# Deci-AI/super-gradients

Measured on NVIDIA H100. Metric: images/sec YOLO-NAS-S 640 bf16 train, higher is better.
Workload: dtype bf16

## Files before the change

include/sgb200.h:

```cpp
#ifndef SGB200_H_
#define SGB200_H_

#include <stdint.h>

#ifdef __cplusplus
extern "C" {
#endif

#define SGB_OK 0
#define SGB_E_INVALID (-1)
#define SGB_E_UNSUPPORTED (-2)
#define SGB_E_CUDA (-3)
#define SGB_E_ARCH (-4)

#define SGB_ACT_NONE 0
#define SGB_ACT_RELU 1
#define SGB_ACT_SILU 2

typedef uint16_t sgb_bf16;

typedef struct SgbConvDesc {
  int32_t N, H, W, C;
  int32_t K, R, S;
  int32_t P, Q;
  int32_t stride, pad;
  int32_t x_pitch, x_off;
  int32_t y_pitch, y_off;
  int32_t up2;
  int32_t centre_from;
} SgbConvDesc;

typedef struct SgbEpilogue {
  const float* scale;
  const float* shift;
  const sgb_bf16* residual;
  double* stats;
  int32_t stats_repl;
  int32_t act;
  int32_t out_f32;
} SgbEpilogue;

const char* sgb_last_error(void);
int sgb_version(void);
int sgb_check_device(void);
int64_t sgb_sm100_launches(void);
int64_t sgb_conv_halo_launches(void);
void sgb_conv_force_im2col(int on);
int64_t sgb_conv_wgrad_halo_launches(void);
void sgb_conv_wgrad_force_im2col(int on);

int sgb_conv_fprop(const SgbConvDesc* d, const sgb_bf16* x, const sgb_bf16* w_krsc, void* y, const SgbEpilogue* ep,
                   void* stream);
int sgb_conv_dgrad(const SgbConvDesc* d, const sgb_bf16* dy, const sgb_bf16* w_crsk, sgb_bf16* dx, int accumulate,
                   void* stream);
int sgb_conv_wgrad(const SgbConvDesc* d, const sgb_bf16* x, const sgb_bf16* dy, float* dw_krsc, void* stream);
int sgb_weight_prepare(const float* w_oihw, int K, int C, int R, int S, int c_pad, sgb_bf16* w_krsc, sgb_bf16* w_crsk,
                       const float* scale, int add_identity, void* stream);
int sgb_wgrad_to_oihw(const float* dw_krsc, int K, int C, int R, int S, int c_pad, float* g_oihw, int accumulate,
                      void* stream);
typedef struct SgbWeightItem {
  const float* w;
  const float* scale;
  sgb_bf16* krsc;
  sgb_bf16* crsk;
  int32_t K, C, R, S, c_pad, add_identity;
  int32_t kp, koff, etaps, etap;
  int64_t start;
} SgbWeightItem;
typedef struct SgbWgradItem {
  const float* dw;
  float* g;
  int32_t K, C, R, S, c_pad, accumulate;
  int64_t start;
} SgbWgradItem;
int sgb_weight_prepare_batch(const SgbWeightItem* items_dev, int n_items, int64_t total, void* stream);
typedef struct SgbAlphaItem {
  const float* dw1;
  const float* w1;
  const float* alpha;
  const float* dab;
  const float* bias1;
  float* g_w1;
  float* g_bias;
  float* g_alpha;
  int32_t K, C, c_pad, pad_;
} SgbAlphaItem;
int sgb_qarep_alpha_finish_batch(const SgbAlphaItem* items_dev, int n_items, void* stream);
int sgb_wgrad_to_oihw_batch(const SgbWgradItem* items_dev, int n_items, int64_t total, void* stream);
int sgb_convt2x2_fprop(const SgbConvDesc* d, const sgb_bf16* x_small, const sgb_bf16* w_up, const float* bias,
                       sgb_bf16* y_up, void* stream);

int sgb_nchw_f32_to_nhwc_bf16(const float* x, int N, int C, int H, int W, sgb_bf16* y, int y_pitch, int y_off, int c_out,
                              void* stream);
int sgb_stem_patches_f32(const float* x, int N, int C, int H, int W, int R, int stride, int pad, sgb_bf16* y, int P, int Q, int c_out,
                         void* stream);
int sgb_nhwc_bf16_to_nchw_f32(const sgb_bf16* x, int N, int C, int H, int W, int x_pitch, int x_off, float* y,
                              void* stream);

typedef struct SgbBnDesc {
  int64_t M;
  int32_t C;
  int32_t x_pitch, x_off;
  int32_t y_pitch, y_off;
  int32_t r_pitch, r_off;
  float eps, momentum;
  int32_t act;
  int32_t stats_repl;
  int32_t dy_pitch, dy_off;
  int64_t hw;
  const float* sample_scale;
  int32_t dy2_split, dy2_pitch, dy2_off, dy2_reserved;
  const void* dy2;
  const double* count;
  float param_scale;
  int32_t count_reserved;
} SgbBnDesc;
int sgb_bn_act_fwd(const SgbBnDesc* d, const sgb_bf16* x, const double* stats, const float* gamma, const float* beta,
                   float* running_mean, float* running_var, const sgb_bf16* residual, sgb_bf16* y, float* save_mean,
                   float* save_rstd, void* stream);
int sgb_bn_act_infer(const SgbBnDesc* d, const sgb_bf16* x, const float* gamma, const float* beta,
                     const float* running_mean, const float* running_var, const sgb_bf16* residual, sgb_bf16* y,
                     void* stream);
int sgb_bn_act_bwd_reduce(const SgbBnDesc* d, const sgb_bf16* dy, const sgb_bf16* x, const sgb_bf16* y, const float* gamma,
                          const float* beta, const float* save_mean, const float* save_rstd, double* sums, void* stream);
int sgb_bn_act_bwd_apply(const SgbBnDesc* d, const sgb_bf16* dy, const sgb_bf16* x, const sgb_bf16* y,
                         const float* gamma, const float* beta, const float* save_mean, const float* save_rstd,
                         const double* sums, sgb_bf16* dx, sgb_bf16* dresidual, float* dgamma, float* dbeta, void* stream);
int sgb_channel_stats(const sgb_bf16* x, int64_t M, int C, int pitch, int off, double* stats, void* stream);

typedef struct SgbQarepDesc {
  int64_t M;
  int32_t C;
// ... 295 lines not shown
```

super_gradients_b200/csrc/capi.cu:

```cuda
#include <cstdarg>
#include <cstdio>

#include "common.cuh"
#include "conv_sm100.h"
#include "sm100_host.h"

static thread_local char g_err[512] = "";

void sgb_set_error(const char* fmt, ...) {
  va_list ap;
  va_start(ap, fmt);
  vsnprintf(g_err, sizeof(g_err), fmt, ap);
  va_end(ap);
}

int sgb_cuda_check(cudaError_t e, const char* what) {
  if (e == cudaSuccess) return SGB_OK;
  sgb_set_error("%s: %s", what, cudaGetErrorString(e));
  return SGB_E_CUDA;
}

extern "C" const char* sgb_last_error(void) { return g_err; }
extern "C" int sgb_version(void) { return 100; }
extern "C" int sgb_check_device(void) {
  int dev = 0;
  if (int rc = sgb_cuda_check(cudaGetDevice(&dev), "cudaGetDevice")) return rc;
  cudaDeviceProp prop;
  if (int rc = sgb_cuda_check(cudaGetDeviceProperties(&prop, dev), "cudaGetDeviceProperties")) return rc;
  if (prop.major != 9) {
    sgb_set_error("libsgb200 is built for sm_90a only; device is sm_%d%d", prop.major, prop.minor);
    return SGB_E_ARCH;
  }
  return SGB_OK;
}

extern "C" int64_t sgb_sm100_launches(void) { return (int64_t)sm100::launch_count(); }
extern "C" int64_t sgb_conv_halo_launches(void) { return (int64_t)sm100::halo_launch_count(); }
extern "C" void sgb_conv_force_im2col(int on) { sm100::force_im2col(on != 0); }
extern "C" int64_t sgb_conv_wgrad_halo_launches(void) { return (int64_t)sm100::wgrad_halo_launch_count(); }
extern "C" void sgb_conv_wgrad_force_im2col(int on) { sm100::wgrad_force_im2col(on != 0); }
```

super_gradients_b200/csrc/conv_sm100.cu:

```cuda
#include <cuda.h>

#include <cstdlib>
#include <cstring>

#include "common.cuh"
#include "conv_sm100.h"
#include "sm100_host.h"
#include "sm100_ptx.cuh"

namespace sm100 {

constexpr int BLOCK_M = 128;
constexpr int NUM_THREADS = 384;
constexpr int CONSUMER_THREADS = 256;
constexpr int MAX_STAGES = 8;

struct Params {
  int M;
  int N;
  int C;
  int KC;
  int n_tiles;
  int stages;
  int P, Q;
// ... 289 lines not shown
    asm volatile("fence.mbarrier_init.release.cluster;" ::: "memory");
    asm volatile("fence.proxy.async.shared::cta;" ::: "memory");
  }
  if (p.stats)
    for (int i = threadIdx.x; i < 4 * p.N; i += NUM_THREADS) s_stats[i] = 0.f;
  __syncthreads();

  if (warp == 0) {
    if (elect_one()) {
      mbar_expect_tx(b_bar, (uint32_t)(8 * off + ksteps) * b_box);
      for (int bt = 0; bt < 9; ++bt)
        for (int ks = 0; ks < (bt == CENTRE_TAP ? ksteps : off); ++ks)
          tma_load_2d(sb + (uint32_t)(bt * ksteps + ks) * b_box, &map_b, b_bar, bt * p.b_cols_per_tap + 16 * ks, nt * BN);
      const uint32_t a_tx = (uint32_t)(p.C / 8) * (HALO_H * HALO_W * 16);
      int stg = 0;
      uint32_t par = 1;
      for (int mt = mt0; mt < m_tiles; mt += mt_step) {
        const int n_img = mt / p.halo_thw;
        const int rem = mt - n_img * p.halo_thw;
        const int th = rem / p.halo_tw, tw = rem - th * p.halo_tw;
        mbar_wait(empty_bar(stg), par);
        const uint32_t sa = sa0 + stg * a_stage;
        mbar_expect_tx(full_bar(stg), a_tx);
        for (int cg = 0; cg < p.C / 8; ++cg)
          tma_load_tiled_4d(sa + (uint32_t)cg * HALO_CG_BYTES, &map_a, full_bar(stg), 8 * cg, tw * HALO_TILE - 1, th * HALO_TILE - 1,
                            n_img);
        if (++stg == p.stages) {
          stg = 0;
          par ^= 1;
        }
      }
    }
  } else if (warp >= 4) {
    const int wg = (warp >> 2) - 1;
    const int wq = warp & 3;
    float acc[BN / 2];
    mbar_wait(b_bar, 0);
    for (int j = wg, mt = mt0 + wg * mt_step; mt < m_tiles; j += 2, mt += 2 * mt_step) {
      const int stg = j % p.stages;
      mbar_wait(full_bar(stg), (uint32_t)(j / p.stages) & 1u);
      const uint32_t sa = sa0 + stg * a_stage;
      wgmma_fence();
      int t = off > 0 ? 0 : CENTRE_TAP;
      uint32_t sa_t = sa + (uint32_t)((t / 3) * HALO_W + t % 3) * 16u, sb_t = sb + (uint32_t)(p.tap_b[t] * ksteps) * b_box;
      for (int k = 0, ks = 0, nk = 8 * off + ksteps; k < nk; ++k) {
        const uint64_t da = smem_desc_noswizzle(sa_t + (uint32_t)(2 * ks) * HALO_CG_BYTES, HALO_CG_BYTES, HALO_W * 16);
        const uint64_t db = smem_desc(sb_t + (uint32_t)ks * b_box, 32, 16u, 256u);
        mma_kk<BN>(acc, da, db, k != 0);
        if (++ks == (t == CENTRE_TAP ? ksteps : off) && ++t < 9) {
          ks = 0;
          sa_t = sa + (uint32_t)((t / 3) * HALO_W + t % 3) * 16u;
          sb_t = sb + (uint32_t)(p.tap_b[t] * ksteps) * b_box;
        }
      }
      wgmma_commit();
      wgmma_wait<0>();
      fence_regs(acc);
      __syncwarp();
      if (lane == 0) mbar_arrive(empty_bar(stg));

      const int n_img = mt / p.halo_thw;
      const int rem = mt - n_img * p.halo_thw;
      const int th = rem / p.halo_tw, tw = rem - th * p.halo_tw;
      const int ow = tw * HALO_TILE + (lane >> 2);
      long long orow[2];
      bool row_ok[2];
#pragma unroll
      for (int h = 0; h < 2; ++h) {
        const int oh = th * HALO_TILE + 2 * wq + h;
        row_ok[h] = oh < p.P && ow < p.Q;
        orow[h] = row_ok[h] ? ((long long)n_img * p.P + oh) * p.Q + ow : 0;
      }
      tile_epilogue<BN, 4>(p, acc, orow, row_ok, nt, wg, wq, lane, s_part + wg * 4 * 2 * BN, s_stats + wg * 2 * p.N);
    }
  }
  __syncthreads();
  if (p.stats) {
    for (int i = threadIdx.x; i < 2 * p.N; i += NUM_THREADS) s_stats[i] += s_stats[2 * p.N + i];
    __syncthreads();
  }
  flush_stats(p, s_stats);
}

struct WParams {
  int K, C;
  int R, S, stride, pad, P, Q;
  int npix;
  int CB;
  int n_ctiles;
  int rb_all, rb_off;
  int items;
  int pix_per_cta;
  int stages;
  int cpad;
  float* dw;
  int halo_tw, halo_thw, tiles, tiles_per_cta;
};
constexpr int WPIX = 64;

__host__ __device__ __forceinline__ int wgrad_row_blocks(const WParams& p, int tap) {
  return p.R * p.S == 9 && tap != CENTRE_TAP ? p.rb_off : p.rb_all;
}

template <int NB>
__global__ void __launch_bounds__(NUM_THREADS, 1)
wgrad_wgmma_kernel(const __grid_constant__ CUtensorMap map_dy, const __grid_constant__ CUtensorMap map_x, const WParams p) {
  extern __shared__ __align__(1024) unsigned char smem_raw[];
  const uint32_t smem_base = (smem_u32(smem_raw) + 1023u) & ~1023u;
  const uint32_t a_bytes = 2 * WPIX * 128;
  const uint32_t b_box = WPIX * p.CB * 2;
  const int boxes = NB / p.CB;
  const uint32_t stage_bytes = a_bytes + (uint32_t)boxes * b_box;
  const uint32_t ctrl = smem_base + p.stages * stage_bytes;
  auto full_bar = [&](int s) { return ctrl + 8u * s; };
  auto empty_bar = [&](int s) { return ctrl + 8u * (MAX_STAGES + s); };

  const int warp = threadIdx.x >> 5, lane = threadIdx.x & 31;
  int w = blockIdx.x;
  const int split = w / (p.items * p.n_ctiles);
  w -= split * p.items * p.n_ctiles;
  int tap = 0, tap_items = (wgrad_row_blocks(p, 0) + 1) / 2;
  while (w >= tap_items * p.n_ctiles) {
    w -= tap_items * p.n_ctiles;
    tap_items = (wgrad_row_blocks(p, ++tap) + 1) / 2;
  }
  const int ctile = w / tap_items, item = w - ctile * tap_items;
  const bool shared_rows = 2 * item + 1 == wgrad_row_blocks(p, tap);
  const int row0 = 128 * item;
  const int pix0 = split * p.pix_per_cta;
  const int pix1 = min(pix0 + p.pix_per_cta, p.npix);
  const int n_iters = (pix1 - pix0 + WPIX - 1) / WPIX;

  if (threadIdx.x == 0) {
    for (int s = 0; s < p.stages; ++s) {
      mbar_init(full_bar(s), 1);
      mbar_init(empty_bar(s), shared_rows ? 4 : 8);
    }
    asm volatile("fence.mbarrier_init.release.cluster;" ::: "memory");
    asm volatile("fence.proxy.async.shared::cta;" ::: "memory");
  }
  __syncthreads();

  if (n_iters > 0) {
    if (warp == 0) {
      if (elect_one()) {
        const int pq = p.P * p.Q;
        const int r = tap / p.S, s = tap - r * p.S;
        int stg = 0;
        uint32_t par = 1;
        for (int it = 0; it < n_iters; ++it) {
          mbar_wait(empty_bar(stg), par);
          const uint32_t sa = smem_base + stg * stage_bytes, sb = sa + a_bytes;
          mbar_expect_tx(full_bar(stg), (shared_rows ? a_bytes / 2 : a_bytes) + (uint32_t)boxes * b_box);
          const int pix = pix0 + it * WPIX;
          tma_load_2d(sa, &map_dy, full_bar(stg), row0, pix);
          if (!shared_rows) tma_load_2d(sa + WPIX * 128, &map_dy, full_bar(stg), row0 + 64, pix);
          const int n_img = pix / pq;
          const int rem = pix - n_img * pq;
          const int p0 = rem / p.Q, q0 = rem - p0 * p.Q;
          const int w0 = q0 * p.stride - p.pad, h0 = p0 * p.stride - p.pad;
          for (int bx = 0; bx < boxes; ++bx)
            tma_load_im2col_4d(sb + (uint32_t)bx * b_box, &map_x, full_bar(stg), ctile * NB + bx * p.CB, w0, h0, n_img, (uint16_t)s,
                               (uint16_t)r);
          if (++stg == p.stages) {
            stg = 0;
            par ^= 1;
// ... 107 lines not shown
      if (ko < p.K) {
        float* drow = p.dw + (long long)ko * row_len + tap0 * p.cpad + ctile * NB + 2 * (lane & 3);
#pragma unroll
        for (int t = 0; t < NT; ++t)
#pragma unroll
          for (int j = 0; j < NB / 8; ++j)
            asm volatile("red.global.add.v2.f32 [%0], {%1, %2};" ::"l"(drow + t * p.cpad + 8 * j), "f"(acc[t][4 * j + 2 * h]),
                         "f"(acc[t][4 * j + 2 * h + 1])
                         : "memory");
      }
    }
  }
}

template <int NB>
__global__ void __launch_bounds__(NUM_THREADS, 1)
wgrad3x3_halo_kernel(const __grid_constant__ CUtensorMap map_dy, const __grid_constant__ CUtensorMap map_x, const WParams p) {
  extern __shared__ __align__(1024) unsigned char smem_raw[];
  const uint32_t smem_base = (smem_u32(smem_raw) + 1023u) & ~1023u;
  constexpr uint32_t a_bytes = WH_A_BYTES, stage_bytes = wgrad_halo_stage_bytes(NB);
  const uint32_t ctrl = smem_base + p.stages * stage_bytes;
  auto full_bar = [&](int s) { return ctrl + 8u * s; };
  auto empty_bar = [&](int s) { return ctrl + 8u * (MAX_STAGES + s); };

  const int warp = threadIdx.x >> 5;
  const int items = p.rb_all * p.n_ctiles;
  const int split = blockIdx.x / items, item = blockIdx.x - split * items;
  const int ctile = item / p.rb_all, rb = item - ctile * p.rb_all;
  const bool all_taps = rb < p.rb_off;
  const int t0 = split * p.tiles_per_cta, t1 = min(t0 + p.tiles_per_cta, p.tiles);

  if (threadIdx.x == 0) {
    for (int s = 0; s < p.stages; ++s) {
      mbar_init(full_bar(s), 1);
      mbar_init(empty_bar(s), 8);
    }
    asm volatile("fence.mbarrier_init.release.cluster;" ::: "memory");
    asm volatile("fence.proxy.async.shared::cta;" ::: "memory");
  }
  __syncthreads();

  if (warp == 0) {
    if (elect_one()) {
      const uint32_t tx = a_bytes + (NB / 8) * (HALO_H * HALO_W * 16);
      int stg = 0;
      uint32_t par = 1;
      for (int mt = t0; mt < t1; ++mt) {
        const int n_img = mt / p.halo_thw;
        const int rem = mt - n_img * p.halo_thw;
        const int th = rem / p.halo_tw, tw = rem - th * p.halo_tw;
        mbar_wait(empty_bar(stg), par);
        const uint32_t sa = smem_base + stg * stage_bytes;
        mbar_expect_tx(full_bar(stg), tx);
        tma_load_tiled_4d(sa, &map_dy, full_bar(stg), 64 * rb, tw * HALO_TILE, th * HALO_TILE, n_img);
        for (int cg = 0; cg < NB / 8; ++cg)
          tma_load_tiled_4d(sa + a_bytes + (uint32_t)cg * HALO_CG_BYTES, &map_x, full_bar(stg), ctile * NB + 8 * cg,
                            tw * HALO_TILE - 1, th * HALO_TILE - 1, n_img);
        if (++stg == p.stages) {
          stg = 0;
          par ^= 1;
        }
      }
    }
  } else if (warp >= 4) {
    const int wg = (warp >> 2) - 1;
    const uint32_t ring = smem_base, bars = ctrl;
    if (!all_taps && wg == 0)
      wgrad_halo_consume<NB, 1>(p, ring, bars, t0, t1, CENTRE_TAP, rb, ctile);
    else if (!all_taps)
      wgrad_halo_consume<NB, 0>(p, ring, bars, t0, t1, 0, rb, ctile);
    else if (wg == 0)
      wgrad_halo_consume<NB, 5>(p, ring, bars, t0, t1, 0, rb, ctile);
    else
      wgrad_halo_consume<NB, 4>(p, ring, bars, t0, t1, 5, rb, ctile);
  }
}

EncodeTiledFn g_tiled = nullptr;
EncodeIm2colFn g_im2col = nullptr;
int g_num_sms = 0;
long long g_launches = 0;
long long g_halo_launches = 0;
long long g_wgrad_halo_launches = 0;
bool g_force_im2col = false;
bool g_wgrad_force_im2col = false;
long long launch_count() { return g_launches; }
long long halo_launch_count() { return g_halo_launches; }
long long wgrad_halo_launch_count() { return g_wgrad_halo_launches; }
void force_im2col(bool on) { g_force_im2col = on; }
void wgrad_force_im2col(bool on) { g_wgrad_force_im2col = on; }

int init_driver() {
  if (g_tiled && g_im2col) return SGB_OK;
  cudaDriverEntryPointQueryResult qres;
  void* fn = nullptr;
  if (cudaGetDriverEntryPoint("cuTensorMapEncodeTiled", &fn, cudaEnableDefault, &qres) != cudaSuccess || !fn) {
    sgb_set_error("cuTensorMapEncodeTiled entry point not found");
    return SGB_E_CUDA;
  }
  g_tiled = (EncodeTiledFn)fn;
  fn = nullptr;
  if (cudaGetDriverEntryPoint("cuTensorMapEncodeIm2col", &fn, cudaEnableDefault, &qres) != cudaSuccess || !fn) {
    sgb_set_error("cuTensorMapEncodeIm2col entry point not found");
    return SGB_E_CUDA;
  }
  g_im2col = (EncodeIm2colFn)fn;
  int dev = 0;
  cudaGetDevice(&dev);
  cudaDeviceGetAttribute(&g_num_sms, cudaDevAttrMultiProcessorCount, dev);
  return SGB_OK;
}

CUtensorMapSwizzle swizzle_for(int kc) {
  return kc == 64 ? CU_TENSOR_MAP_SWIZZLE_128B : (kc == 32 ? CU_TENSOR_MAP_SWIZZLE_64B : CU_TENSOR_MAP_SWIZZLE_32B);
}

bool supported(const Problem& q) {
  if (q.C % 16 != 0 || q.b_rows % 8 != 0) return false;
  if (!((q.R == 1 && q.S == 1) || (q.R == 3 && q.S == 3))) return false;
  if (q.stride != 1 && q.stride != 2) return false;
  if (q.a_pitch % 8 != 0 || q.y_pitch % 8 != 0 || q.y_off % 8 != 0) return false;
  if (((uintptr_t)q.a & 15) || ((uintptr_t)q.b & 15) || ((uintptr_t)q.y & 15)) return false;
  if ((long long)q.N * q.P * q.Q >= (1ll << 31)) return false;
  if (q.b_rows > 4096) return false;
  return true;
}

namespace {

template <class Fn>
struct Variant {
  int bn;
  Fn fn;
  int regs;
  bool ready;
};
typedef void (*ConvFn)(const CUtensorMap, const CUtensorMap, const Params);
typedef void (*WgradFn)(const CUtensorMap, const CUtensorMap, const WParams);
Variant<ConvFn> g_conv[] = {{16, conv_wgmma_kernel<16, false>, 0, false},   {32, conv_wgmma_kernel<32, false>, 0, false},
                            {48, conv_wgmma_kernel<48, false>, 0, false},   {64, conv_wgmma_kernel<64, false>, 0, false},
                            {96, conv_wgmma_kernel<96, false>, 0, false},   {128, conv_wgmma_kernel<128, false>, 0, false}};
Variant<ConvFn> g_conv_skip[] = {{16, conv_wgmma_kernel<16, true>, 0, false},   {32, conv_wgmma_kernel<32, true>, 0, false},
                                 {48, conv_wgmma_kernel<48, true>, 0, false},   {64, conv_wgmma_kernel<64, true>, 0, false},
                                 {96, conv_wgmma_kernel<96, true>, 0, false},   {128, conv_wgmma_kernel<128, true>, 0, false}};
Variant<ConvFn> g_halo[] = {{16, conv3x3_halo_kernel<16, false>, 0, false},   {32, conv3x3_halo_kernel<32, false>, 0, false},
                            {48, conv3x3_halo_kernel<48, false>, 0, false},   {64, conv3x3_halo_kernel<64, false>, 0, false},
                            {96, conv3x3_halo_kernel<96, false>, 0, false},   {128, conv3x3_halo_kernel<128, false>, 0, false}};
Variant<ConvFn> g_halo_skip[] = {{16, conv3x3_halo_kernel<16, true>, 0, false},   {32, conv3x3_halo_kernel<32, true>, 0, false},
                                 {48, conv3x3_halo_kernel<48, true>, 0, false},   {64, conv3x3_halo_kernel<64, true>, 0, false},
                                 {96, conv3x3_halo_kernel<96, true>, 0, false},   {128, conv3x3_halo_kernel<128, true>, 0, false}};
Variant<WgradFn> g_wgrad[] = {{16, wgrad_wgmma_kernel<16>, 0, false}, {32, wgrad_wgmma_kernel<32>, 0, false},
                              {48, wgrad_wgmma_kernel<48>, 0, false}, {64, wgrad_wgmma_kernel<64>, 0, false},
                              {96, wgrad_wgmma_kernel<96>, 0, false}, {128, wgrad_wgmma_kernel<128>, 0, false}};
Variant<WgradFn> g_wgrad_halo[] = {{16, wgrad3x3_halo_kernel<16>, 0, false}, {32, wgrad3x3_halo_kernel<32>, 0, false},
                                   {48, wgrad3x3_halo_kernel<48>, 0, false}};

template <class Fn>
int prepare(Variant<Fn>& v, const char* what) {
  if (v.ready) return SGB_OK;
  if (int rc = sgb_cuda_check(cudaFuncSetAttribute(v.fn, cudaFuncAttributeMaxDynamicSharedMemorySize, 227 * 1024), what)) return rc;
  cudaFuncAttributes fa{};
  if (int rc = sgb_cuda_check(cudaFuncGetAttributes(&fa, v.fn), what)) return rc;
  v.regs = fa.numRegs;
  v.ready = true;
  return SGB_OK;
}

int pick_bn(int n) {
  for (int bn : {16, 32, 48, 64, 96, 128})
    if (n <= bn) return bn;
  int best = 128, best_waste = (n + 127) / 128 * 128 - n;
  for (int bn : {96, 64}) {
    const int waste = (n + bn - 1) / bn * bn - n;
    if (waste < best_waste) { best_waste = waste; best = bn; }
  }
  return best;
}

size_t halo_smem(int C, int bn, int n, bool stats, int stages) {
  const size_t b_bytes = ((size_t)9 * C * bn * 2 + 1023) & ~(size_t)1023;
  const size_t a_stage = ((size_t)(C / 8) * HALO_CG_BYTES + 1023) & ~(size_t)1023;
  return 1024 + b_bytes + (size_t)stages * a_stage + HALO_CTRL_BYTES + (stats ? (size_t)(8 * 2 * bn + 4 * n) * 4 : 0);
}

bool halo_tiles_fit(int P, int Q) {
  const long long covered = (long long)((P + 7) / 8) * 8 * ((Q + 7) / 8) * 8;
  return 20ll * P * Q >= 17 * covered;
}

int halo_bn(const Problem& q) {
  if (q.R != 3 || q.S != 3 || q.stride != 1 || q.pad != 1 || q.ntaps > 0 || q.out_mode != 0) return 0;
  if (q.P != q.H || q.Q != q.W) return 0;
  if (!halo_tiles_fit(q.P, q.Q)) return 0;
  const int n = q.b_rows, full = pick_bn(n);
  auto waste = [&](int bn) { return (n + bn - 1) / bn * bn - n; };
  for (int bn : {full, 96, 64})
    if (bn <= full && (bn == full || (q.C <= 96 && bn >= 64 && waste(bn) <= waste(full))) &&
        halo_smem(q.C, bn, n, q.stats != nullptr, 2) <= 227 * 1024)
      return bn;
  return 0;
}

int encode_halo_map(CUtensorMap* map, const void* x, int N, int H, int W, int C, int pitch) {
  cuuint64_t dims[4] = {(cuuint64_t)C, (cuuint64_t)W, (cuuint64_t)H, (cuuint64_t)N};
  cuuint64_t strides[3] = {(cuuint64_t)pitch * 2, (cuuint64_t)W * pitch * 2, (cuuint64_t)H * W * pitch * 2};
  cuuint32_t box[4] = {8, HALO_W, HALO_H, 1};
  cuuint32_t estr[4] = {1, 1, 1, 1};
  CUresult r = g_tiled(map, CU_TENSOR_MAP_DATA_TYPE_BFLOAT16, 4, const_cast<void*>(x), dims, strides, box, estr, CU_TENSOR_MAP_INTERLEAVE_NONE,
                       CU_TENSOR_MAP_SWIZZLE_NONE, CU_TENSOR_MAP_L2_PROMOTION_L2_128B, CU_TENSOR_MAP_FLOAT_OOB_FILL_NONE);
  if (r != CUDA_SUCCESS) {
    sgb_set_error("cuTensorMapEncodeTiled(halo) failed with %d (C=%d W=%d H=%d N=%d pitch=%d)", (int)r, C, W, H, N, pitch);
    return SGB_E_CUDA;
  }
  return SGB_OK;
}

int launch_halo(const Problem& q, const Params& p0, int bn, cudaStream_t st) {
  Params p = p0;
  p.n_tiles = (p.N + bn - 1) / bn;
  p.halo_tw = (q.Q + HALO_TILE - 1) / HALO_TILE;
  p.halo_thw = p.halo_tw * ((q.P + HALO_TILE - 1) / HALO_TILE);
  p.M = q.N * p.halo_thw;
  p.centre_n = 0;
  Variant<ConvFn>* var = nullptr;
  for (auto& v : p.centre_c > 0 ? g_halo_skip : g_halo)
    if (v.bn == bn) var = &v;
  if (int rc = prepare(*var, "conv3x3_halo_kernel")) return rc;
  const int regs_alloc = ((var->regs + 7) / 8) * 8 * NUM_THREADS;
  int ctas_per_sm = 65536 / regs_alloc;
  if (ctas_per_sm > 2) ctas_per_sm = 2;
  if (ctas_per_sm < 1) ctas_per_sm = 1;
  int stages = 0;
  for (;; --ctas_per_sm) {
    const size_t budget = (ctas_per_sm == 1 ? 227u : 227u / ctas_per_sm - 1u) * 1024u;
    for (stages = HALO_MAX_STAGES; stages >= 2 && halo_smem(q.C, bn, p.N, p.stats != nullptr, stages) > budget; --stages) {
    }
    if (stages >= 2 || ctas_per_sm == 1) break;
  }
  if (stages < 2) { sgb_set_error("conv3x3_halo: tile does not fit shared memory"); return SGB_E_UNSUPPORTED; }
  p.stages = stages;
  const size_t smem = halo_smem(q.C, bn, p.N, p.stats != nullptr, stages);

  alignas(64) CUtensorMap map_a, map_b;
  if (int rc = encode_halo_map(&map_a, q.a, q.N, q.H, q.W, q.C, q.a_pitch)) return rc;
  {
    cuuint64_t dims[2] = {(cuuint64_t)q.b_cols, (cuuint64_t)q.b_rows};
    cuuint64_t strides[1] = {(cuuint64_t)q.b_cols * 2};
    cuuint32_t box[2] = {16, (cuuint32_t)bn};
    cuuint32_t estr[2] = {1, 1};
    CUresult r = g_tiled(&map_b, CU_TENSOR_MAP_DATA_TYPE_BFLOAT16, 2, const_cast<void*>(q.b), dims, strides, box, estr,
                         CU_TENSOR_MAP_INTERLEAVE_NONE, CU_TENSOR_MAP_SWIZZLE_32B, CU_TENSOR_MAP_L2_PROMOTION_L2_128B,
                         CU_TENSOR_MAP_FLOAT_OOB_FILL_NONE);
    if (r != CUDA_SUCCESS) {
      sgb_set_error("cuTensorMapEncodeTiled(halo B) failed with %d (cols=%d rows=%d BN=%d)", (int)r, q.b_cols, q.b_rows, bn);
      return SGB_E_CUDA;
    }
  }
  int per_nt = g_num_sms * ctas_per_sm / p.n_tiles;
  if (per_nt > p.M) per_nt = p.M;
  if (per_nt < 1) per_nt = 1;
  var->fn<<<per_nt * p.n_tiles, NUM_THREADS, smem, st>>>(map_a, map_b, p);
  ++g_launches;
  ++g_halo_launches;
  return sgb_cuda_check(cudaGetLastError(), "conv3x3_halo_kernel");
}

}

int launch(const Problem& q, cudaStream_t st) {
  if (int rc = init_driver()) return rc;
  Params p{};
  p.M = q.N * q.P * q.Q;
  p.N = q.b_rows;
  p.C = q.C;
  p.KC = q.C % 64 == 0 ? 64 : (q.C % 32 == 0 ? 32 : 16);
  if (p.KC < 64 && q.C > 32) p.KC = 64;
  const int bn = pick_bn(p.N);
  p.n_tiles = (p.N + bn - 1) / bn;
  p.P = q.P; p.Q = q.Q; p.stride = q.stride; p.pad = q.pad;
  if (q.ntaps > 0) {
    p.ntaps = q.ntaps;
    for (int t = 0; t < q.ntaps; ++t) { p.tap_dh[t] = (signed char)q.tap_dh[t]; p.tap_dw[t] = (signed char)q.tap_dw[t]; p.tap_b[t] = (signed char)q.tap_b[t]; }
  } else {
    p.ntaps = q.R * q.S;
    for (int t = 0; t < p.ntaps; ++t) {
      p.tap_dh[t] = (signed char)(t / q.S);
      p.tap_dw[t] = (signed char)(t % q.S);
      p.tap_b[t] = (signed char)(q.flip ? (p.ntaps - 1 - t) : t);
    }
  }
  if (p.ntaps > 9) return SGB_E_UNSUPPORTED;
  p.out_mode = q.out_mode; p.o_mul = q.o_mul; p.oh_add = q.oh_add; p.ow_add = q.ow_add; p.outH = q.outH; p.outW = q.outW;
  p.b_cols_per_tap = q.b_cols_per_tap;
  p.y = (bf16*)q.y; p.y_pitch = q.y_pitch; p.y_off = q.y_off;
  p.scale = q.scale; p.shift = q.shift; p.residual = (const bf16*)q.residual;
  p.stats = q.stats; p.stats_repl = q.stats_repl > 0 ? q.stats_repl : 1; p.act = q.act;
  if (q.centre_from > 0) {
    if (q.R != 3 || q.S != 3 || q.stride != 1 || q.pad != 1 || q.ntaps > 0 || q.centre_from % 16 != 0 ||
        q.centre_from >= (q.flip ? q.C : q.b_rows))
      return SGB_E_INVALID;
    (q.flip ? p.centre_c : p.centre_n) = q.centre_from;
  }
  if (!g_force_im2col)
    if (const int hbn = halo_bn(q)) return launch_halo(q, p, hbn, st);
  Variant<ConvFn>* var = nullptr;
  for (auto& v : p.centre_n > 0 || p.centre_c > 0 ? g_conv_skip : g_conv)
    if (v.bn == bn) var = &v;
  if (int rc = prepare(*var, "conv_wgmma_kernel")) return rc;
  const uint32_t a_bytes = BLOCK_M * p.KC * 2, b_bytes = ((uint32_t)(bn * p.KC * 2) + 1023u) & ~1023u;
  const uint32_t stage_bytes = a_bytes + b_bytes;
  const uint32_t ctrl_bytes = CTRL_BAR_BYTES + (p.stats ? (uint32_t)(8 * 2 * bn + 2 * p.N) * 4u : 0u);
  const int regs_alloc = ((var->regs + 7) / 8) * 8 * NUM_THREADS;
  int ctas_per_sm = 65536 / regs_alloc;
  if (ctas_per_sm > 2) ctas_per_sm = 2;
  if (ctas_per_sm < 1) ctas_per_sm = 1;
  int stages = 0;
  for (;; --ctas_per_sm) {
    const uint32_t budget = (ctas_per_sm == 1 ? 226u : 227u / ctas_per_sm - 1u) * 1024u;
    stages = budget > ctrl_bytes + 1024 ? (int)((budget - ctrl_bytes - 1024) / stage_bytes) : 0;
    if (stages > MAX_STAGES) stages = MAX_STAGES;
    if (stages >= 4 || ctas_per_sm == 1) break;
  }
  if (stages < 2) { sgb_set_error("conv_wgmma: tile does not fit shared memory"); return SGB_E_UNSUPPORTED; }
  p.stages = stages;
  const size_t smem = 1024 + (size_t)stages * stage_bytes + ctrl_bytes;

  alignas(64) CUtensorMap map_a, map_b;
  {
    cuuint64_t dims[4] = {(cuuint64_t)q.C, (cuuint64_t)q.W, (cuuint64_t)q.H, (cuuint64_t)q.N};
    cuuint64_t strides[3] = {(cuuint64_t)q.a_pitch * 2, (cuuint64_t)q.W * q.a_pitch * 2, (cuuint64_t)q.H * q.W * q.a_pitch * 2};
    int lower[2] = {-q.pad, -q.pad};
    int upper[2] = {q.pad - (q.S - 1), q.pad - (q.R - 1)};
    if (q.ntaps > 0) {
      lower[0] = lower[1] = 0;
      upper[0] = q.Q - q.W;
      upper[1] = q.P - q.H;
    }
    cuuint32_t estr[4] = {1, (cuuint32_t)q.stride, (cuuint32_t)q.stride, 1};
    CUresult r = g_im2col(&map_a, CU_TENSOR_MAP_DATA_TYPE_BFLOAT16, 4, const_cast<void*>(q.a), dims, strides, lower, upper,
                          (cuuint32_t)p.KC, (cuuint32_t)BLOCK_M, estr, CU_TENSOR_MAP_INTERLEAVE_NONE, swizzle_for(p.KC),
                          CU_TENSOR_MAP_L2_PROMOTION_L2_128B, CU_TENSOR_MAP_FLOAT_OOB_FILL_NONE);
    if (r != CUDA_SUCCESS) {
      sgb_set_error("cuTensorMapEncodeIm2col failed with %d (C=%d W=%d H=%d N=%d pitch=%d pad=%d upper=%d,%d stride=%d KC=%d)", (int)r,
                    q.C, q.W, q.H, q.N, q.a_pitch, q.pad, upper[0], upper[1], q.stride, p.KC);
      return SGB_E_CUDA;
    }
  }
  {
    cuuint64_t dims[2] = {(cuuint64_t)q.b_cols, (cuuint64_t)q.b_rows};
    cuuint64_t strides[1] = {(cuuint64_t)q.b_cols * 2};
    cuuint32_t box[2] = {(cuuint32_t)p.KC, (cuuint32_t)bn};
    cuuint32_t estr[2] = {1, 1};
    CUresult r = g_tiled(&map_b, CU_TENSOR_MAP_DATA_TYPE_BFLOAT16, 2, const_cast<void*>(q.b), dims, strides, box, estr,
                         CU_TENSOR_MAP_INTERLEAVE_NONE, swizzle_for(p.KC), CU_TENSOR_MAP_L2_PROMOTION_L2_128B,
                         CU_TENSOR_MAP_FLOAT_OOB_FILL_NONE);
    if (r != CUDA_SUCCESS) {
      sgb_set_error("cuTensorMapEncodeTiled(B) failed with %d (cols=%d rows=%d KC=%d BN=%d)", (int)r, q.b_cols, q.b_rows, p.KC, bn);
      return SGB_E_CUDA;
    }
  }
  const int m_tiles = (p.M + BLOCK_M - 1) / BLOCK_M;
  int grid = m_tiles * p.n_tiles;
  if (grid > g_num_sms * ctas_per_sm) grid = g_num_sms * ctas_per_sm;
  var->fn<<<grid, NUM_THREADS, smem, st>>>(map_a, map_b, p);
  ++g_launches;
  return sgb_cuda_check(cudaGetLastError(), "conv_wgmma_kernel");
}

bool wgrad_supported(const WgradProblem& q) {
  if (q.C % 16 != 0 || q.K % 8 != 0) return false;
  if (!((q.R == 1 && q.S == 1) || (q.R == 3 && q.S == 3))) return false;
  if (q.pad != q.R / 2 || (q.stride != 1 && q.stride != 2)) return false;
  if (q.x_pitch % 8 != 0 || q.y_pitch % 8 != 0) return false;
  if (((uintptr_t)q.x & 15) || ((uintptr_t)q.dy & 15)) return false;
  if ((long long)q.N * q.P * q.Q >= (1ll << 31)) return false;
  return true;
}

namespace {

int wgrad_halo_nb(const WgradProblem& q) {
  if (q.R != 3 || q.S != 3 || q.stride != 1 || q.pad != 1 || q.P != q.H || q.Q != q.W) return 0;
  if (!halo_tiles_fit(q.P, q.Q)) return 0;
  return q.C % 32 == 0 ? 32 : (q.C % 48 == 0 ? 48 : 16);
}

int launch_wgrad_halo(const WgradProblem& q, const WParams& p0, int nb, cudaStream_t st) {
// ... 116 lines not shown
```

super_gradients_b200/csrc/conv_sm100.h:

```cpp
#pragma once
#include <cuda_runtime.h>

namespace sm100 {

struct Problem {
  const void* a;
  int N, H, W, C, a_pitch;
  const void* b;
  int b_rows, b_cols, b_cols_per_tap;
  int R, S, stride, pad, P, Q, flip;
  int ntaps;
  int tap_dh[9], tap_dw[9], tap_b[9];
  int out_mode, o_mul, oh_add, ow_add, outH, outW;
  void* y;
  int y_pitch, y_off;
  const float* scale;
  const float* shift;
  const void* residual;
  double* stats;
  int stats_repl, act;
  int centre_from;
};

struct WgradProblem {
  const void* x;
  const void* dy;
  int N, H, W, C, x_pitch;
  int K, y_pitch;
  int R, S, stride, pad, P, Q;
  float* dw;
  int centre_from;
};

bool wgrad_supported(const WgradProblem& q);
int wgrad_launch(const WgradProblem& q, cudaStream_t st);
bool supported(const Problem& q);
int launch(const Problem& q, cudaStream_t st);
long long launch_count();
long long halo_launch_count();
void force_im2col(bool on);
long long wgrad_halo_launch_count();
void wgrad_force_im2col(bool on);

}
```

super_gradients_b200/lib.py:

```python
import ctypes
import os
from ctypes import POINTER, Structure, c_char_p, c_double, c_float, c_int, c_int32, c_int64, c_void_p

_HERE = os.path.dirname(os.path.abspath(__file__))
LIB_PATH = os.path.join(_HERE, "libsgb200.so")

ACT_NONE, ACT_RELU, ACT_SILU = 0, 1, 2


class SgbError(RuntimeError):
    pass


class ConvDesc(Structure):
    _fields_ = [(n, c_int32) for n in ("N", "H", "W", "C", "K", "R", "S", "P", "Q", "stride", "pad", "x_pitch", "x_off", "y_pitch", "y_off", "up2", "centre_from")]


class Epilogue(Structure):
    _fields_ = [
        ("scale", c_void_p),
        ("shift", c_void_p),
        ("residual", c_void_p),
        ("stats", c_void_p),
        ("stats_repl", c_int32),
# ... 53 lines not shown
        ("offu", c_int32),
        ("pitcho", c_int32),
        ("offo", c_int32),
        ("eps3", c_float),
        ("eps_post", c_float),
        ("momentum", c_float),
        ("act", c_int32),
        ("use_post_bn", c_int32),
        ("pitchd", c_int32),
        ("offd", c_int32),
        ("pitchr", c_int32),
        ("offr", c_int32),
        ("res", c_void_p),
        ("res_alpha", c_void_p),
        ("count", c_void_p),
        ("param_scale", c_float),
        ("count_reserved", c_int32),
    ]


class PoseLossDesc(Structure):
    _fields_ = (
        [(n, c_int32) for n in ("B", "L", "J", "reg_max", "n_max", "topk")]
        + [(n, c_float) for n in ("alpha", "beta", "w_cls", "w_iou", "w_dfl", "w_pose_cls", "w_pose_reg")]
        + [(n, c_int32) for n in ("iou_type", "cls_type", "pose_cls_type", "multiply_by_oks", "rescale_with_score")]
    )


class PreprocDesc(Structure):
    _fields_ = (
        [(n, c_int32) for n in ("src_h", "src_w", "src_c", "src_pitch", "dst_h", "dst_w", "out_h", "out_w", "pad_top", "pad_left", "out_pitch", "reverse_channels", "normalize")]
        + [("pad_value", c_float), ("max_value", c_double), ("mean", c_float * 4), ("std", c_float * 4)]
    )


class MatchDesc(Structure):
    _fields_ = [(n, c_int32) for n in ("B", "max_preds", "max_targets", "max_crowd", "n_thresholds", "top_k", "denormalize_targets")] + [("height", c_float), ("width", c_float)]


class LossDesc(Structure):
    _fields_ = [
        ("B", c_int32),
        ("L", c_int32),
        ("ncls", c_int32),
        ("reg_max", c_int32),
        ("n_max", c_int32),
        ("topk", c_int32),
        ("alpha", c_float),
        ("beta", c_float),
        ("w_cls", c_float),
        ("w_iou", c_float),
        ("w_dfl", c_float),
        ("iou_type", c_int32),
    ]


class NmsDesc(Structure):
    _fields_ = [
        ("B", c_int32),
        ("L", c_int32),
        ("ncls", c_int32),
        ("score_thr", c_float),
        ("iou_thr", c_double),
        ("top_k", c_int32),
        ("max_out", c_int32),
        ("multi_label", c_int32),
        ("class_agnostic", c_int32),
        ("thr_inclusive", c_int32),
    ]


P = c_void_p
_I, _F, _L = c_int, c_float, c_int64

_SIGNATURES = {
    "sgb_last_error": (c_char_p, []),
    "sgb_version": (c_int, []),
    "sgb_check_device": (c_int, []),
    "sgb_sm100_launches": (c_int64, []),
    "sgb_conv_halo_launches": (c_int64, []),
    "sgb_conv_force_im2col": (None, [_I]),
    "sgb_conv_wgrad_halo_launches": (c_int64, []),
    "sgb_conv_wgrad_force_im2col": (None, [_I]),
    "sgb_conv_fprop": (c_int, [POINTER(ConvDesc), P, P, P, POINTER(Epilogue), P]),
    "sgb_conv_dgrad": (c_int, [POINTER(ConvDesc), P, P, P, _I, P]),
    "sgb_conv_wgrad": (c_int, [POINTER(ConvDesc), P, P, P, P]),
    "sgb_weight_prepare": (c_int, [P, _I, _I, _I, _I, _I, P, P, P, _I, P]),
    "sgb_wgrad_to_oihw": (c_int, [P, _I, _I, _I, _I, _I, P, _I, P]),
    "sgb_weight_prepare_batch": (c_int, [P, _I, c_int64, P]),
    "sgb_wgrad_to_oihw_batch": (c_int, [P, _I, c_int64, P]),
    "sgb_qarep_alpha_finish_batch": (c_int, [P, _I, P]),
    "sgb_convt2x2_fprop": (c_int, [POINTER(ConvDesc), P, P, P, P, P]),
    "sgb_nchw_f32_to_nhwc_bf16": (c_int, [P, _I, _I, _I, _I, P, _I, _I, _I, P]),
    "sgb_stem_patches_f32": (c_int, [P, _I, _I, _I, _I, _I, _I, _I, P, _I, _I, _I, P]),
    "sgb_nhwc_bf16_to_nchw_f32": (c_int, [P, _I, _I, _I, _I, _I, _I, P, P]),
    "sgb_bn_act_fwd": (c_int, [POINTER(BnDesc), P, P, P, P, P, P, P, P, P, P, P]),
    "sgb_bn_act_fwd_fused": (c_int, [POINTER(BnDesc), P, P, P, P, P, P, P, P, P, P, P]),
    "sgb_bn_act_infer": (c_int, [POINTER(BnDesc), P, P, P, P, P, P, P, P]),
    "sgb_bn_act_bwd_reduce": (c_int, [POINTER(BnDesc), P, P, P, P, P, P, P, P, P]),
    "sgb_bn_act_bwd_apply": (c_int, [POINTER(BnDesc), P, P, P, P, P, P, P, P, P, P, P, P, P]),
    "sgb_bn_act_bwd_fused": (c_int, [POINTER(BnDesc), P, P, P, P, P, P, P, P, P, P, P, P, P]),
    "sgb_channel_stats": (c_int, [P, _L, _I, _I, _I, P, P]),
    "sgb_qarep_moments": (c_int, [POINTER(QarepDesc), P, P, P, P]),
    "sgb_qarep_fwd": (c_int, [POINTER(QarepDesc)] + [P] * 15),
    "sgb_qarep_fwd_fused": (c_int, [POINTER(QarepDesc)] + [P] * 15),
    "sgb_qarep_bwd_reduce": (c_int, [POINTER(QarepDesc), P, P, P, P, P, P, P]),
    "sgb_qarep_bwd_apply": (c_int, [POINTER(QarepDesc)] + [P] * 16),
    "sgb_qarep_bwd_fused": (c_int, [POINTER(QarepDesc)] + [P] * 15),
    "sgb_maxpool_fwd": (c_int, [P, _I, _I, _I, _I, _I, _I, _I, _I, _I, P, _I, _I, _I, _I, P, P]),
    "sgb_maxpool_bwd": (c_int, [P, _I, _I, _I, _I, _I, _I, _I, _I, _I, _I, _I, P, P, P]),
    "sgb_maxpool_bwd_bf16": (c_int, [P, _I, _I, _I, _I, _I, _I, _I, _I, _I, _I, _I, P, P, _I, P]),
    "sgb_axpby": (c_int, [P, _I, _I, _F, P, _I, _I, _F, P, _I, _I, _L, _I, P]),
    "sgb_scale_add": (c_int, [P, _I, _I, P, P, _I, _I, P, _I, _I, _L, _I, P]),
    "sgb_channel_dot": (c_int, [P, _I, _I, P, _I, _I, _L, _I, P, P]),
    "sgb_scale_add_dot": (c_int, [P, _I, _I, P, P, _I, _I, P, _I, _I, P, _I, _I, _L, _I, P, P]),
    "sgb_f32_to_bf16": (c_int, [P, P, _L, P]),
    "sgb_avgpool_fwd": (c_int, [P, _I, _I, _I, P, P]),
    "sgb_avgpool_bwd": (c_int, [P, _I, _I, _I, P, P]),
    "sgb_dfl_decode": (c_int, [P, _I, P, _I, _I, _I, _I, _I, _I, _I, _I, _F, _F, P, P, P, P, P]),
    "sgb_pose_keypoint_decode": (c_int, [P, _I, P, _I, _I, _I, _I, _I, _I, _I, _I, _F, _F, _F, _I, P, P, P, P]),
    "sgb_tal_assign": (c_int, [POINTER(LossDesc)] + [P] * 12 + [_L, P]),
    "sgb_tal_workspace_bytes": (c_int64, [POINTER(LossDesc)]),
    "sgb_atss_assign": (c_int, [POINTER(LossDesc)] + [P] * 5 + [c_int32] + [P] * 7 + [P, _L, P]),
    "sgb_atss_workspace_bytes": (c_int64, [POINTER(LossDesc)]),
    "sgb_dfl_iou_loss_fwd_bwd": (c_int, [POINTER(LossDesc)] + [P] * 8 + [_F, P, P, P]),
    "sgb_focal_cls_fwd_bwd": (c_int, [POINTER(LossDesc), P, P, P, P, c_float, c_float, P, P]),
    "sgb_loss_finalize": (c_int, [POINTER(LossDesc), P, P, P]),
    "sgb_preprocess_u8": (c_int, [POINTER(PreprocDesc), P, P, P]),
    "sgb_resample_crop_u8": (c_int, [P, P, P, _L, _I, _I, _I, _I, _I, _I, c_double, P, P, P, P]),
    "sgb_classify_rows": (c_int, [P, _L, _I, _L, _I, P, P, _L, _I, _I, P, P, P, P]),
    "sgb_detection_augment": (c_int, [P, P, P, _L, _I, _I, _I, _I, _I, _I, c_double, _I, P, P]),
    "sgb_pose_augment": (c_int, [P, P, P, _L, P, _L, _I, _I, _I, c_double, _I, P, P]),
    "sgb_detection_matching": (c_int, [POINTER(MatchDesc), P, P, P, P, P, P, P, P, P, P]),
    "sgb_pose_keypoint_matching": (c_int, [P] * 10 + [_I] * 6 + [P] * 7),
    "sgb_pose_tal_workspace_bytes": (c_int64, [POINTER(PoseLossDesc)]),
    "sgb_pose_tal_assign": (c_int, [POINTER(PoseLossDesc)] + [P] * 14 + [_L, P]),
    "sgb_pose_loss_fwd_bwd": (c_int, [POINTER(PoseLossDesc)] + [P] * 12 + [_F] + [P] * 5),
    "sgb_pose_loss_finalize": (c_int, [POINTER(PoseLossDesc), P, P, P]),
    "sgb_head_grad_scatter": (c_int, [P, _I, _I, _I, _I, _I, P, _I, P]),
    "sgb_sliding_window_gather": (c_int, [P, _I, _I, _I, _I, P, P, _I, _I, P, P]),
    "sgb_sliding_window_merge_workspace_bytes": (c_int64, [_I, P, _I, _I, _I]),
    "sgb_sliding_window_merge": (c_int, [P, P, P, P, P, _I, _I, _I, _I, c_double, P, P, P, _L, P]),
    "sgb_sliding_window_merge_launches": (c_int32, [_I, P, _I, _I]),
    "sgb_nms_workspace_bytes": (c_int64, [POINTER(NmsDesc)]),
    "sgb_batched_nms": (c_int, [POINTER(NmsDesc), P, P, P, P, P, P, _L, P]),
    "sgb_sgd_step": (c_int, [P, P, P, _L, P, P]),
    "sgb_adamw_step": (c_int, [P, P, P, P, _L, P, P]),
    "sgb_ema_update": (c_int, [P, P, _L, P, P]),
}

_lib = None

LAUNCH_COUNT = {"sgb_tal_assign": 4, "sgb_atss_assign": 3, "sgb_pose_tal_assign": 4, "sgb_sm100_launches": 0, "sgb_conv_halo_launches": 0, "sgb_conv_force_im2col": 0, "sgb_conv_wgrad_halo_launches": 0, "sgb_conv_wgrad_force_im2col": 0, "sgb_sliding_window_merge_workspace_bytes": 0, "sgb_sliding_window_merge_launches": 0, "sgb_last_error": 0, "sgb_version": 0, "sgb_check_device": 0}
LAUNCHES = [0]


def exported_names():
    return sorted(_SIGNATURES)


def load():
    global _lib
    if _lib is not None:
        return _lib
    if not os.path.exists(LIB_PATH):
        raise SgbError(f"{LIB_PATH} not found: run `python -c 'import __graft_entry__ as g; g.build()'` " "(there is no non-CUDA fallback for this package)")
    lib = ctypes.CDLL(LIB_PATH)
    for name, (res, args) in _SIGNATURES.items():
        fn = getattr(lib, name)
        fn.restype = res
        fn.argtypes = args
    _lib = lib
    return lib


def check(rc, what=""):
    if rc != 0:
        msg = load().sgb_last_error()
        raise SgbError(f"{what} failed with code {rc}: {msg.decode() if msg else ''}")


def call(name, *args):
    lib = load()
    rc = getattr(lib, name)(*args)
    LAUNCHES[0] += LAUNCH_COUNT.get(name, 1)
    if rc != 0:
        msg = lib.sgb_last_error()
        raise SgbError(f"{name} failed with code {rc}: {msg.decode() if msg else ''}")
```

Baseline: 946.3.

## Add persistent 1x1 conv kernel with shared-memory-resident filter slice

Adds a dedicated persistent WGMMA kernel for stride-1 unpadded 1x1 convolutions without stats. Each CTA loads its whole filter slice into shared memory once with TMA, then streams 64-row activation tiles through two per-warpgroup rings. This avoids reloading weights for every M tile. The trade-offs are a large shared-memory footprint that can reduce stages or occupancy, and the path is skipped when BN statistics are fused, which limits how often it applies in training.

Result: faster. 956.7 (median of 6 runs) (+1.1%).

```diff
diff --git a/include/sgb200.h b/include/sgb200.h
--- a/include/sgb200.h
+++ b/include/sgb200.h
@@ -48,6 +48,8 @@
 void sgb_conv_force_im2col(int on);
 int64_t sgb_conv_wgrad_halo_launches(void);
 void sgb_conv_wgrad_force_im2col(int on);
+int64_t sgb_conv_1x1_launches(void);
+void sgb_conv_1x1_force_generic(int on);
 
 int sgb_conv_fprop(const SgbConvDesc* d, const sgb_bf16* x, const sgb_bf16* w_krsc, void* y, const SgbEpilogue* ep,
                    void* stream);
diff --git a/super_gradients_b200/csrc/capi.cu b/super_gradients_b200/csrc/capi.cu
--- a/super_gradients_b200/csrc/capi.cu
+++ b/super_gradients_b200/csrc/capi.cu
@@ -39,3 +39,5 @@
 extern "C" void sgb_conv_force_im2col(int on) { sm100::force_im2col(on != 0); }
 extern "C" int64_t sgb_conv_wgrad_halo_launches(void) { return (int64_t)sm100::wgrad_halo_launch_count(); }
 extern "C" void sgb_conv_wgrad_force_im2col(int on) { sm100::wgrad_force_im2col(on != 0); }
+extern "C" int64_t sgb_conv_1x1_launches(void) { return (int64_t)sm100::conv1x1_launch_count(); }
+extern "C" void sgb_conv_1x1_force_generic(int on) { sm100::conv1x1_force_generic(on != 0); }
diff --git a/super_gradients_b200/csrc/conv_sm100.cu b/super_gradients_b200/csrc/conv_sm100.cu
--- a/super_gradients_b200/csrc/conv_sm100.cu
+++ b/super_gradients_b200/csrc/conv_sm100.cu
@@ -395,6 +395,116 @@
   flush_stats(p, s_stats);
 }
 
+constexpr int C1_TILE = 64;
+constexpr uint32_t C1_CTRL_BYTES = 2 * CTRL_BAR_BYTES + 16;
+
+__host__ __device__ constexpr uint32_t c1_filter_bytes(int C, int kc, int bn) {
+  return (uint32_t)((C + kc - 1) / kc) * (((uint32_t)(bn * kc * 2) + 1023u) & ~1023u);
+}
+
+template <int BN>
+__global__ void __launch_bounds__(NUM_THREADS, BN <= 64 ? 2 : 1)
+conv1x1_kernel(const __grid_constant__ CUtensorMap map_a, const __grid_constant__ CUtensorMap map_b, const Params p) {
+  extern __shared__ __align__(1024) unsigned char smem_raw[];
+  const uint32_t smem_base = (smem_u32(smem_raw) + 1023u) & ~1023u;
+  const int chunks = (p.C + p.KC - 1) / p.KC;
+  const uint32_t b_box = ((uint32_t)(BN * p.KC * 2) + 1023u) & ~1023u;
+  const uint32_t a_stage = (uint32_t)(C1_TILE * p.KC * 2);
+  const uint32_t sb = smem_base, sa0 = smem_base + c1_filter_bytes(p.C, p.KC, BN);
+  const uint32_t ctrl = sa0 + 2u * (uint32_t)p.stages * a_stage;
+  auto full_bar = [&](int r, int s) { return ctrl + (uint32_t)r * CTRL_BAR_BYTES + 8u * s; };
+  auto empty_bar = [&](int r, int s) { return ctrl + (uint32_t)r * CTRL_BAR_BYTES + 8u * (MAX_STAGES + s); };
+  const uint32_t b_bar = ctrl + 2 * CTRL_BAR_BYTES;
+
+  const int warp = threadIdx.x >> 5, lane = threadIdx.x & 31;
+  const int m_tiles = (p.M + C1_TILE - 1) / C1_TILE;
+  const int nt = blockIdx.x % p.n_tiles;
+  const int mt_step = gridDim.x / p.n_tiles;
+  const int mt0 = blockIdx.x / p.n_tiles;
+
+  if (threadIdx.x == 0) {
+    for (int r = 0; r < 2; ++r)
+      for (int s = 0; s < p.stages; ++s) {
+        mbar_init(full_bar(r, s), 1);
+        mbar_init(empty_bar(r, s), 4);
+      }
+    mbar_init(b_bar, 1);
+    asm volatile("fence.mbarrier_init.release.cluster;" ::: "memory");
+    asm volatile("fence.proxy.async.shared::cta;" ::: "memory");
+  }
+  __syncthreads();
+
+  if (warp == 0) {
+    if (elect_one()) {
+      mbar_expect_tx(b_bar, (uint32_t)(chunks * BN * p.KC * 2));
+      for (int ck = 0; ck < chunks; ++ck) tma_load_2d(sb + (uint32_t)ck * b_box, &map_b, b_bar, ck * p.KC, nt * BN);
+      int stg[2] = {0, 0};
+      uint32_t par[2] = {1, 1};
+      for (int j = 0, mt = mt0; mt < m_tiles; ++j, mt += mt_step) {
+        const int r = j & 1;
+        for (int ck = 0; ck < chunks; ++ck) {
+          mbar_wait(empty_bar(r, stg[r]), par[r]);
+          mbar_expect_tx(full_bar(r, stg[r]), a_stage);
+          tma_load_2d(sa0 + (uint32_t)(r * p.stages + stg[r]) * a_stage, &map_a, full_bar(r, stg[r]), ck * p.KC, mt * C1_TILE);
+          if (++stg[r] == p.stages) {
+            stg[r] = 0;
+            par[r] ^= 1;
+          }
+        }
+      }
+    }
+  } else if (warp >= 4) {
+    const int wg = (warp >> 2) - 1;
+    const int wq = warp & 3;
+    const int row_bytes = p.KC * 2;
+    const uint32_t sbo = 8u * (uint32_t)row_bytes;
+    const int ksteps = p.KC / 16;
+    const uint32_t ring = sa0 + (uint32_t)(wg * p.stages) * a_stage;
+    float acc[BN / 2];
+    int stg = 0;
+    uint32_t par = 0;
+    mbar_wait(b_bar, 0);
+    for (int mt = mt0 + wg * mt_step; mt < m_tiles; mt += 2 * mt_step) {
+      int prev = -1;
+      for (int ck = 0; ck < chunks; ++ck) {
+        mbar_wait(full_bar(wg, stg), par);
+        const uint32_t sa = ring + (uint32_t)stg * a_stage, sb_ck = sb + (uint32_t)ck * b_box;
+        wgmma_fence();
+        for (int ks = 0; ks < ksteps; ++ks) {
+          const uint64_t da = smem_desc(sa + 32u * ks, row_bytes, 16u, sbo), db = smem_desc(sb_ck + 32u * ks, row_bytes, 16u, sbo);
+          mma_kk<BN>(acc, da, db, (ck | ks) != 0);
+        }
+        wgmma_commit();
+        if (prev >= 0) {
+          wgmma_wait<1>();
+          __syncwarp();
+          if (lane == 0) mbar_arrive(empty_bar(wg, prev));
+        }
+        prev = stg;
+        if (++stg == p.stages) {
+          stg = 0;
+          par ^= 1;
+        }
+      }
+      wgmma_wait<0>();
+      fence_regs(acc);
+      __syncwarp();
+      if (lane == 0) mbar_arrive(empty_bar(wg, prev));
+
+      const long long m_lo = (long long)mt * C1_TILE + wq * 16 + (lane >> 2);
+      long long orow[2];
+      bool row_ok[2];
+#pragma unroll
+      for (int h = 0; h < 2; ++h) {
+        const long long m = m_lo + 8 * h;
+        row_ok[h] = m < p.M;
+        orow[h] = row_ok[h] ? m : 0;
+      }
+      tile_epilogue<BN, 4>(p, acc, orow, row_ok, nt, wg, wq, lane, nullptr, nullptr);
+    }
+  }
+}
+
 struct WParams {
   int K, C;
   int R, S, stride, pad, P, Q;
@@ -668,13 +778,17 @@
 long long g_launches = 0;
 long long g_halo_launches = 0;
 long long g_wgrad_halo_launches = 0;
+long long g_1x1_launches = 0;
 bool g_force_im2col = false;
 bool g_wgrad_force_im2col = false;
+bool g_1x1_force_generic = false;
 long long launch_count() { return g_launches; }
 long long halo_launch_count() { return g_halo_launches; }
 long long wgrad_halo_launch_count() { return g_wgrad_halo_launches; }
+long long conv1x1_launch_count() { return g_1x1_launches; }
 void force_im2col(bool on) { g_force_im2col = on; }
 void wgrad_force_im2col(bool on) { g_wgrad_force_im2col = on; }
+void conv1x1_force_generic(bool on) { g_1x1_force_generic = on; }
 
 int init_driver() {
   if (g_tiled && g_im2col) return SGB_OK;
@@ -740,6 +854,9 @@
                               {96, wgrad_wgmma_kernel<96>, 0, false}, {128, wgrad_wgmma_kernel<128>, 0, false}};
 Variant<WgradFn> g_wgrad_halo[] = {{16, wgrad3x3_halo_kernel<16>, 0, false}, {32, wgrad3x3_halo_kernel<32>, 0, false},
                                    {48, wgrad3x3_halo_kernel<48>, 0, false}};
+Variant<ConvFn> g_1x1[] = {{16, conv1x1_kernel<16>, 0, false}, {32, conv1x1_kernel<32>, 0, false},
+                           {48, conv1x1_kernel<48>, 0, false}, {64, conv1x1_kernel<64>, 0, false},
+                           {96, conv1x1_kernel<96>, 0, false}, {128, conv1x1_kernel<128>, 0, false}};
 
 template <class Fn>
 int prepare(Variant<Fn>& v, const char* what) {
@@ -849,6 +966,81 @@
   ++g_launches;
   ++g_halo_launches;
   return sgb_cuda_check(cudaGetLastError(), "conv3x3_halo_kernel");
+}
+
+size_t c1x1_smem(int C, int kc, int bn, int stages) {
+  return 1024 + (size_t)c1_filter_bytes(C, kc, bn) + (size_t)2 * stages * C1_TILE * kc * 2 + C1_CTRL_BYTES;
+}
+
+int c1x1_bn(const Problem& q, int kc) {
+  if (q.R != 1 || q.S != 1 || q.stride != 1 || q.pad != 0 || q.ntaps > 0 || q.out_mode != 0) return 0;
+  if (q.P != q.H || q.Q != q.W || q.C > 512 || q.stats) return 0;
+  const int n = q.b_rows, full = pick_bn(n);
+  const long long m = (long long)q.N * q.P * q.Q;
+  auto waste = [&](int bn) { return (n + bn - 1) / bn * bn - n; };
+  for (int bn : {full, 96, 64, 48, 32, 16})
+    if (bn <= full && waste(bn) <= waste(full) && c1x1_smem(q.C, kc, bn, 2) <= 227 * 1024)
+      return m * ((n + bn - 1) / bn) >= 4ll * bn * g_num_sms && (q.C <= 384 || bn >= n) ? bn : 0;
+  return 0;
+}
+
+int launch_1x1(const Problem& q, const Params& p0, int bn, cudaStream_t st) {
+  Params p = p0;
+  p.n_tiles = (p.N + bn - 1) / bn;
+  Variant<ConvFn>* var = nullptr;
+  for (auto& v : g_1x1)
+    if (v.bn == bn) var = &v;
+  if (int rc = prepare(*var, "conv1x1_kernel")) return rc;
+  const int regs_alloc = ((var->regs + 7) / 8) * 8 * NUM_THREADS;
+  int ctas_per_sm = 65536 / regs_alloc;
+  if (ctas_per_sm > 2) ctas_per_sm = 2;
+  if (ctas_per_sm < 1) ctas_per_sm = 1;
+  int stages = 0;
+  for (;; --ctas_per_sm) {
+    const size_t budget = (ctas_per_sm == 1 ? 227u : 227u / ctas_per_sm - 1u) * 1024u;
+    for (stages = MAX_STAGES; stages >= 2 && c1x1_smem(q.C, p.KC, bn, stages) > budget; --stages) {
+    }
+    if (stages >= 2 || ctas_per_sm == 1) break;
+  }
+  if (stages < 2) { sgb_set_error("conv1x1: filter slice does not fit shared memory"); return SGB_E_UNSUPPORTED; }
+  p.stages = stages;
+  const size_t smem = c1x1_smem(q.C, p.KC, bn, stages);
+
+  alignas(64) CUtensorMap map_a, map_b;
+  {
+    cuuint64_t dims[2] = {(cuuint64_t)q.C, (cuuint64_t)p.M};
+    cuuint64_t strides[1] = {(cuuint64_t)q.a_pitch * 2};
+    cuuint32_t box[2] = {(cuuint32_t)p.KC, (cuuint32_t)C1_TILE};
+    cuuint32_t estr[2] = {1, 1};
+    CUresult r = g_tiled(&map_a, CU_TENSOR_MAP_DATA_TYPE_BFLOAT16, 2, const_cast<void*>(q.a), dims, strides, box, estr,
+                         CU_TENSOR_MAP_INTERLEAVE_NONE, swizzle_for(p.KC), CU_TENSOR_MAP_L2_PROMOTION_L2_128B,
+                         CU_TENSOR_MAP_FLOAT_OOB_FILL_NONE);
+    if (r != CUDA_SUCCESS) {
+      sgb_set_error("cuTensorMapEncodeTiled(1x1 A) failed with %d (C=%d M=%d pitch=%d KC=%d)", (int)r, q.C, p.M, q.a_pitch, p.KC);
+      return SGB_E_CUDA;
+    }
+  }
+  {
+    cuuint64_t dims[2] = {(cuuint64_t)q.b_cols, (cuuint64_t)q.b_rows};
+    cuuint64_t strides[1] = {(cuuint64_t)q.b_cols * 2};
+    cuuint32_t box[2] = {(cuuint32_t)p.KC, (cuuint32_t)bn};
+    cuuint32_t estr[2] = {1, 1};
+    CUresult r = g_tiled(&map_b, CU_TENSOR_MAP_DATA_TYPE_BFLOAT16, 2, const_cast<void*>(q.b), dims, strides, box, estr,
+                         CU_TENSOR_MAP_INTERLEAVE_NONE, swizzle_for(p.KC), CU_TENSOR_MAP_L2_PROMOTION_L2_128B,
+                         CU_TENSOR_MAP_FLOAT_OOB_FILL_NONE);
+    if (r != CUDA_SUCCESS) {
+      sgb_set_error("cuTensorMapEncodeTiled(1x1 B) failed with %d (cols=%d rows=%d KC=%d BN=%d)", (int)r, q.b_cols, q.b_rows, p.KC, bn);
+      return SGB_E_CUDA;
+    }
+  }
+  const int m_tiles = (p.M + C1_TILE - 1) / C1_TILE;
+  int per_nt = g_num_sms * ctas_per_sm / p.n_tiles;
+  if (per_nt > m_tiles) per_nt = m_tiles;
+  if (per_nt < 1) per_nt = 1;
+  var->fn<<<per_nt * p.n_tiles, NUM_THREADS, smem, st>>>(map_a, map_b, p);
+  ++g_launches;
+  ++g_1x1_launches;
+  return sgb_cuda_check(cudaGetLastError(), "conv1x1_kernel");
 }
 
 }
@@ -889,6 +1081,8 @@
   }
   if (!g_force_im2col)
     if (const int hbn = halo_bn(q)) return launch_halo(q, p, hbn, st);
+  if (!g_1x1_force_generic)
+    if (const int c1bn = c1x1_bn(q, p.KC)) return launch_1x1(q, p, c1bn, st);
   Variant<ConvFn>* var = nullptr;
   for (auto& v : p.centre_n > 0 || p.centre_c > 0 ? g_conv_skip : g_conv)
     if (v.bn == bn) var = &v;
diff --git a/super_gradients_b200/csrc/conv_sm100.h b/super_gradients_b200/csrc/conv_sm100.h
--- a/super_gradients_b200/csrc/conv_sm100.h
+++ b/super_gradients_b200/csrc/conv_sm100.h
@@ -41,5 +41,7 @@
 void force_im2col(bool on);
 long long wgrad_halo_launch_count();
 void wgrad_force_im2col(bool on);
+long long conv1x1_launch_count();
+void conv1x1_force_generic(bool on);
 
 }
diff --git a/super_gradients_b200/lib.py b/super_gradients_b200/lib.py
--- a/super_gradients_b200/lib.py
+++ b/super_gradients_b200/lib.py
@@ -159,6 +159,8 @@
     "sgb_conv_force_im2col": (None, [_I]),
     "sgb_conv_wgrad_halo_launches": (c_int64, []),
     "sgb_conv_wgrad_force_im2col": (None, [_I]),
+    "sgb_conv_1x1_launches": (c_int64, []),
+    "sgb_conv_1x1_force_generic": (None, [_I]),
     "sgb_conv_fprop": (c_int, [POINTER(ConvDesc), P, P, P, POINTER(Epilogue), P]),
     "sgb_conv_dgrad": (c_int, [POINTER(ConvDesc), P, P, P, _I, P]),
     "sgb_conv_wgrad": (c_int, [POINTER(ConvDesc), P, P, P, P]),
@@ -228,7 +230,7 @@
 
 _lib = None
 
-LAUNCH_COUNT = {"sgb_tal_assign": 4, "sgb_atss_assign": 3, "sgb_pose_tal_assign": 4, "sgb_sm100_launches": 0, "sgb_conv_halo_launches": 0, "sgb_conv_force_im2col": 0, "sgb_conv_wgrad_halo_launches": 0, "sgb_conv_wgrad_force_im2col": 0, "sgb_sliding_window_merge_workspace_bytes": 0, "sgb_sliding_window_merge_launches": 0, "sgb_last_error": 0, "sgb_version": 0, "sgb_check_device": 0}
+LAUNCH_COUNT = {"sgb_tal_assign": 4, "sgb_atss_assign": 3, "sgb_pose_tal_assign": 4, "sgb_sm100_launches": 0, "sgb_conv_halo_launches": 0, "sgb_conv_force_im2col": 0, "sgb_conv_wgrad_halo_launches": 0, "sgb_conv_wgrad_force_im2col": 0, "sgb_conv_1x1_launches": 0, "sgb_conv_1x1_force_generic": 0, "sgb_sliding_window_merge_workspace_bytes": 0, "sgb_sliding_window_merge_launches": 0, "sgb_last_error": 0, "sgb_version": 0, "sgb_check_device": 0}
 LAUNCHES = [0]
 
 
```
